# AustenLamacraft/audio-mps

Measured on AMD Instinct MI355X. Metric: audio samples/sec (fwd+bwd) at D=32, T=16000, higher is better.
Workload: dtype f32; 1 GPU; BASELINE configs[2]: PsiCMPS fwd+bwd scan, D=32, T=16000, batch 1024 per GPU (global 1024), input damped_sine, full optimiser step (device-resident chain rule + Adam); parallelism=dp1, kernel_variant=2, kernel_family=wave, input=damped_sine, optimizer_step=device (cmps_psi_apply_step), rank1_updates=f16x2

## Files before the change

audio_mps_amd/build.py:

```python
from __future__ import annotations

import os
import shutil
import subprocess
import sys

_HERE = os.path.dirname(os.path.abspath(__file__))
CSRC = os.path.join(_HERE, "csrc")
LIB_DIR = os.path.join(_HERE, "lib")
LIB_PATH = os.path.join(LIB_DIR, "libcmps.so")
OBJ_DIR = os.path.join(_HERE, "obj")
SOURCES = ["cmps_capi.hip", "cmps_prep.hip", "cmps_opt.hip", "cmps_block.hip", "cmps_wave.hip", "cmps_wave_bwd2.hip", "cmps_wave2.hip", "cmps_wave16.hip", "cmps_pair.hip", "cmps_wide.hip", "cmps_legacy.hip", "cmps_rho.hip", "cmps_rho_wave.hip", "cmps_rho_mfma.hip"]
EXTRA_FLAGS = {"cmps_pair.hip": ["-fno-slp-vectorize"]}
HEADERS = ["cmps_internal.h", "cmps_wave_util.h", "cmps_grad_gemm.h", os.path.join("..", "..", "include", "cmps.h")]


def _hipcc() -> str:
    for cand in (shutil.which("hipcc"), "/opt/rocm/bin/hipcc"):
        if cand and os.path.exists(cand):
            return cand
    raise RuntimeError("hipcc not found: libcmps.so cannot be built")


def needs_build() -> bool:
    if not os.path.exists(LIB_PATH):
        return True
    t = os.path.getmtime(LIB_PATH)
    deps = [os.path.join(CSRC, s) for s in SOURCES + HEADERS]
    return any(os.path.getmtime(d) > t for d in deps if os.path.exists(d))


def _flags():
    return ["--offload-arch=gfx950", "-O3", "-std=c++17", "-fPIC", "-Xarch_host", "-msse4.2", "-Wall", "-Wno-unused-function"]


def _stamp_text(flags) -> str:
    return " ".join(flags) + " | " + " ; ".join(f"{k}: {' '.join(v)}" for k, v in sorted(EXTRA_FLAGS.items()))


def build(force: bool = False, verbose: bool = False, extra_flags=(), jobs: int | None = None) -> str:
    import hashlib
    flags = _flags() + list(extra_flags)
    obj_dir, lib_path = OBJ_DIR, LIB_PATH
    if extra_flags:
        tag = hashlib.sha1(" ".join(extra_flags).encode()).hexdigest()[:10]
        obj_dir, lib_path = OBJ_DIR + "_diag_" + tag, os.path.join(LIB_DIR, f"libcmps_diag_{tag}.so")
    stamp = os.path.join(obj_dir, "flags.txt")
    same_flags = os.path.exists(stamp) and open(stamp).read() == _stamp_text(flags)
    if not force and not extra_flags and same_flags and not needs_build():
        return LIB_PATH
    os.makedirs(LIB_DIR, exist_ok=True)
    os.makedirs(obj_dir, exist_ok=True)
    hipcc = _hipcc()
    hdr_t = max(os.path.getmtime(os.path.join(CSRC, h)) for h in HEADERS if os.path.exists(os.path.join(CSRC, h)))
    todo, objs = [], []
    for s in SOURCES:
        src, obj = os.path.join(CSRC, s), os.path.join(obj_dir, s.replace(".hip", ".o"))
        objs.append(obj)
        if force or not same_flags or not os.path.exists(obj) or os.path.getmtime(obj) < max(os.path.getmtime(src), hdr_t):
            todo.append((src, obj))

    def compile_one(job):
        src, obj = job
        tmp = f"{obj}.{os.getpid()}.tmp"
        cmd = [hipcc] + flags + EXTRA_FLAGS.get(os.path.basename(src), []) + ["-c", src, "-o", tmp]
        if verbose:
            print(" ".join(cmd), file=sys.stderr)
        proc = subprocess.run(cmd, stdout=subprocess.PIPE, stderr=subprocess.STDOUT, text=True)
        if proc.returncode == 0:
            os.replace(tmp, obj)
        return src, proc

    from concurrent.futures import ThreadPoolExecutor
    with ThreadPoolExecutor(max_workers=jobs or min(6, os.cpu_count() or 2)) as pool:
        for src, proc in pool.map(compile_one, todo):
            if proc.returncode != 0:
                raise RuntimeError(f"hipcc failed on {src}:\n" + proc.stdout)
            if verbose and proc.stdout:
                print(proc.stdout, file=sys.stderr)
    with open(stamp, "w") as f:
        f.write(_stamp_text(flags))
    tmp_lib = f"{lib_path}.{os.getpid()}.tmp"
    proc = subprocess.run([hipcc, "--offload-arch=gfx950", "-shared", "-fPIC", "-o", tmp_lib] + objs,
                          stdout=subprocess.PIPE, stderr=subprocess.STDOUT, text=True)
    if proc.returncode != 0:
        raise RuntimeError("hipcc link failed:\n" + proc.stdout)
    os.replace(tmp_lib, lib_path)
    return lib_path


if __name__ == "__main__":
    print(build(force="--force" in sys.argv, verbose=True))
```

audio_mps_amd/csrc/cmps_wave_bwd2.hip:

```cpp
#include "cmps_wave_util.h"

namespace cmps {

namespace {

struct Pre2 {
    float yh, yho, yhp, un, pre;
    v2f rho;
    v2f sd;
    float inv, ten, rad;
};

constexpr int RING_SLOT = 256;
constexpr int RING_VAL = 8 * RING_SLOT;
constexpr int RING_HALF = 3 * RING_VAL;
constexpr int SPIN_MAX = 1 << 22;
constexpr int MT = 4;

__device__ __forceinline__ int flag_load2(unsigned addr) {
    int v;
    asm volatile("ds_read_b32 %0, %1\n\ts_waitcnt lgkmcnt(0)" : "=v"(v) : "v"(addr) : "memory");
    return __builtin_amdgcn_readfirstlane(v);
}
__device__ __forceinline__ void flag_store2(unsigned addr_l, int v) {
    asm volatile("ds_write_b32 %0, %1" : : "v"(addr_l), "v"(v) : "memory");
}
__device__ __forceinline__ void swap_fill(float& a, float& b, v2f& m0, v2f r0, v2f q0, v2f& m1, v2f r1, v2f q1, v2f s2) {
    asm("v_pk_fma_f32 %2, %4, %8, %5 op_sel_hi:[1,0,1]\n\t"
        "v_pk_fma_f32 %3, %6, %8, %7 op_sel_hi:[1,0,1]\n\t"
        "v_permlane32_swap_b32 %0, %1"
        : "+v"(a), "+v"(b), "=&v"(m0), "=&v"(m1) : "v"(r0), "v"(q0), "v"(r1), "v"(q1), "v"(s2));
}
template <int OFF>
__device__ __forceinline__ void ring_write(unsigned addr, float v) {
    asm volatile("ds_write_b32 %0, %1 offset:%2" : : "v"(addr), "v"(v), "n"(OFF) : "memory");
}
__device__ __forceinline__ float wave_max(float x) {
    asm("s_nop 1\n\tv_max_f32_dpp %0, %0, %0 quad_perm:[1,0,3,2] row_mask:0xf bank_mask:0xf\n\t"
        "s_nop 1\n\tv_max_f32_dpp %0, %0, %0 quad_perm:[2,3,0,1] row_mask:0xf bank_mask:0xf\n\t"
        "s_nop 1\n\tv_max_f32_dpp %0, %0, %0 row_half_mirror row_mask:0xf bank_mask:0xf\n\t"
        "s_nop 1\n\tv_max_f32_dpp %0, %0, %0 row_mirror row_mask:0xf bank_mask:0xf\n\t"
        "s_nop 1\n\tv_max_f32_dpp %0, %0, %0 row_bcast:15 row_mask:0xa bank_mask:0xf\n\t"
        "s_nop 1\n\tv_max_f32_dpp %0, %0, %0 row_bcast:31 row_mask:0xc bank_mask:0xf" : "+v"(x));
    return rdlane(x, 63);
}

}

__global__ __launch_bounds__(128 * WAVES, 1) void k_bwd_wave2w(Dev P, const float* __restrict__ audio) {
    __shared__ __attribute__((aligned(16))) float4 stY[WAVES][CHB * 32];
    __shared__ __attribute__((aligned(16))) float4 stR[WAVES][CHB * 16];
    __shared__ __attribute__((aligned(16))) float4 scl[WAVES][CH * 2];
    __shared__ __attribute__((aligned(16))) float2 bcB[WAVES][DPW];
    __shared__ __attribute__((aligned(16))) float ring[WAVES][2 * 3 * 8 * 64];
    __shared__ __attribute__((aligned(8))) float2 sct[WAVES][2][CH];
    __shared__ int flags[WAVES][2];
    __shared__ int flag_sink[WAVES][2][64];
    const int wv = __builtin_amdgcn_readfirstlane(threadIdx.x >> 6), lane = threadIdx.x & 63;
    const int w = wv & (WAVES - 1), role = wv / WAVES;
    const int i = lane & 31, h = lane >> 5;
    const bool hb = h != 0;
    if (threadIdx.x < 2 * WAVES) (&flags[0][0])[threadIdx.x] = 0;
    __syncthreads();
    const int b = blockIdx.x * WAVES + w;
    if (b >= P.B) return;
    const int N = P.N, T = P.T, NC = (N + CH - 1) / CH;
    const int u_top = (N - 1) & 7, a_oct = (N - 1 - u_top) >> 3, n_oct = (u_top ? 1 : 0) + a_oct + 1;
    const unsigned aProd = lds_addr(&flags[w][0]), aCons = lds_addr(&flags[w][1]);
    const unsigned aProdL = lane == 0 ? aProd : lds_addr(&flag_sink[w][0][lane]), aConsL = lane == 0 ? aCons : lds_addr(&flag_sink[w][1][lane]);
    const unsigned aRing0 = lds_addr(&ring[w][0]) + lane * 4;
    const int vr = P.phi0 ? P.phi_rank : 1;
    const int bc = b / vr, av = b - bc * vr;
    const float* xrow = audio + (size_t)bc * T;
    const float* sc = P.scal + scal_off(bc, NC, 0);
    const float A = dev_A(P);
    float* slab = P.slabs + (size_t)b * P.slab_floats;
    constexpr int DD = DPW * DPW;

    if (role == 0) {
        __builtin_amdgcn_s_setprio(3);
        stagger(w);
        v2f MRd[16], MQ[16], MM[16];
#pragma unroll
        for (int m = 0; m < 16; ++m) {
            const v2f rt = ld2(&P.RT[i * DPW + 16 * h + m]);
            MRd[m] = mk2(rt.x, -rt.y);
            MQ[m] = ld2(&P.Q[i * DPW + 16 * h + m]);
        }
        const unsigned aBw = lds_addr(&bcB[w][0]) + i * 8 + h * 4, aBr = lds_addr(&bcB[w][0]) + h * 128;
        const unsigned aYown = lds_addr(&stY[w][0]) + (2 * i + h) * 8;
        const unsigned aRho = lds_addr(&stR[w][0]) + i * 8;
        const unsigned aScl = lds_addr(&scl[w][0]);
        const float4* rho4 = reinterpret_cast<const float4*>(P.rho);
        const float4* sty4 = reinterpret_cast<const float4*>(P.hst + ((size_t)bc * N * vr + av) * 128);
        float facc = 0.f, accS = 0.f, accA = 0.f;
        float ra0 = 0.f, ra1 = 0.f, rdt = 0.f, rnv = 1.f, rev = 0.f;
        v4f so4[4], so2[2];
        auto octet_load = [&](int hh, int q) {
            stage_load512<4>(sty4, hh * CHB + 8 * q, N - 1, lane, so4, vr);
            stage_load<2>(rho4, hh * CHB + 8 * q, N, lane, so2);
        };
        const unsigned so_lane16 = (unsigned)lane * 16u;
        auto octet_load_below = [&](int hh, int q) {
            if (vr == 1) {
                const int row0 = __builtin_amdgcn_readfirstlane(hh * CHB + 8 * q);
                const float4* py = sty4 + (size_t)row0 * 32;
                const float4* pr = rho4 + (size_t)row0 * 16;
                asm volatile("global_load_dwordx4 %0, %6, %7\n\tglobal_load_dwordx4 %1, %6, %7 offset:1024\n\t"
                             "global_load_dwordx4 %2, %6, %7 offset:2048\n\tglobal_load_dwordx4 %3, %6, %7 offset:3072\n\t"
                             "global_load_dwordx4 %4, %6, %8\n\tglobal_load_dwordx4 %5, %6, %8 offset:1024"
                             : "=&v"(so4[0]), "=&v"(so4[1]), "=&v"(so4[2]), "=&v"(so4[3]), "=&v"(so2[0]), "=&v"(so2[1])
                             : "v"(so_lane16), "s"(py), "s"(pr) : "memory");
            } else {
                octet_load(hh, q);
            }
        };
        auto octet_commit = [&](int q) {
            stage_commit<4>(&stY[w][q * 256], lane, so4);
            stage_commit<2>(&stR[w][q * 128], lane, so2);
        };
        auto octet_commit_below = [&](int q) {
            asm volatile("s_waitcnt vmcnt(0)" : "+v"(so4[0]), "+v"(so4[1]), "+v"(so4[2]), "+v"(so4[3]), "+v"(so2[0]), "+v"(so2[1]) : : "memory");
            octet_commit(q);
        };
        auto scal_load = [&](int c) {
            const int idx = c * CH + lane;
            ra0 = idx < T ? xrow[idx] : 0.f;
            ra1 = idx + 1 < T ? xrow[idx + 1] : 0.f;
            rdt = P.dtk[idx];
            rnv = sc[(size_t)c * 128 + lane];
            rev = sc[(size_t)c * 128 + 64 + lane];
        };
        auto scal_commit = [&](int c) {
            const int idx = c * CH + lane;
            const float inc = ra1 - ra0;
            const float nv = rnv, ev = rev;
            const float invv = rsq_nr(fmaxf(nv, 1e-12f));
            const float invokv = nv > 1e-12f ? invv : 0.f;
            const float sv = inc / A;
            const float ex = ev * inc;
            const float z = ex / A;
            const float zbar = -1.0f / (1.0f + z);
            const float ebar = zbar * inc / A;
            const float tev = 2.0f * ebar;
            scl[w][2 * lane] = make_float4(sv, rdt, invv, tev * nv);
            scl[w][2 * lane + 1] = make_float4(tev, invokv, tev * ev, 0.f);
            sct[w][c & 1][lane] = make_float2(sv, tev * nv);
            if (idx < N) accA += zbar * ex;
        };
        auto make_pre = [&](v2f yh2, v2f rho, v4f c0, v4f c1, v2f sfill) -> Pre2 {
            const float yown = yh2.x, hown = yh2.y;
            Pre2 S;
            S.rho = rho;
            S.sd = __builtin_shufflevector(c0, c0, 0, 1);
            S.inv = c0.z;
            S.ten = c0.w;
            const float te = c1.x;
            const float invok = c1.y;
            S.rad = c1.z;
            S.pre = te * hown;
            S.yh = S.inv * yown;
            S.yhp = invok * yown;
            {
                float ya = S.yh, yb = S.yh;
                swap_fill(ya, yb, MM[10], MRd[10], MQ[10], MM[11], MRd[11], MQ[11], sfill);
                S.yho = hb ? -ya : yb;
            }
            const v2f un = cmul2(mk2(S.yh, S.yho), rho);
            S.un = un.x;
            return S;
        };

        const int hl = (N - 1) / CHB;
#pragma unroll 1
        for (int q = 0; q < 4; ++q) { octet_load(hl, q); octet_commit(q); }
        scal_load(hl >> 1);
        scal_commit(hl >> 1);
        v4f qc[8];
        v2f yh_j, rho_j;
        v4f c0_j, c1_j;
        Pre2 S;
        {
            const int jr = (N - 1) & (CHB - 1), jc = (N - 1) & (CH - 1);
            own_issue(aYown + jr * 512, aRho + jr * 256, aScl + jc * 32, yh_j, rho_j, c0_j, c1_j);
            lds_wait_own<0>(yh_j, rho_j, c0_j, c1_j);
            S = make_pre(yh_j, rho_j, c0_j, c1_j, __builtin_shufflevector(c0_j, c0_j, 0, 1));
        }
        {
            const v2f s2 = mk2(S.sd.x, S.sd.x);
#pragma unroll
            for (int m = 16 - MT; m < 16; ++m) MM[m] = __builtin_elementwise_fma(MRd[m], s2, MQ[m]);
        }
        float g = 0.f, go = 0.f;
        const float2 p0 = P.phi0 ? P.phi0[av * DPW + i] : P.psi0[i];
        const float u0 = hb ? p0.y : p0.x;
        float rad_next = 0.f;

        auto chain_step = [&](const Pre2& S, float uk, auto have_pre, bool exact, unsigned aslot, auto slot_off) -> Pre2 {
            constexpr int SO = decltype(slot_off)::value;
            facc += S.sd.y * (go * S.un);
            const v2f yhbp = cmul2_conj_b(mk2(g, go), S.rho);
            const float yhb = yhbp.x;
            float dot = rad_next;
            if (exact) {
                asm volatile("" ::: "memory");
                dot = sum64(S.yhp * yhb);
            }
            rad_next = S.rad;
            const float ybar = (yhb - dot * S.yhp) * S.inv + S.pre;
            bcast_issue(aBw, aBr, ybar, qc);
            {
                const v2f s2 = mk2(S.sd.x, S.sd.x);
#pragma unroll
                for (int m = 0; m < 16 - MT - 2; ++m) MM[m] = __builtin_elementwise_fma(MRd[m], s2, MQ[m]);
            }
            Pre2 Sn = S;
            if constexpr (!decltype(have_pre)::value) {
                const v2f s2 = mk2(S.sd.x, S.sd.x);
                MM[10] = __builtin_elementwise_fma(MRd[10], s2, MQ[10]);
                MM[11] = __builtin_elementwise_fma(MRd[11], s2, MQ[11]);
            }
            if constexpr (decltype(have_pre)::value) {
                lds_wait_own<9>(yh_j, rho_j, c0_j, c1_j);
                Sn = make_pre(yh_j, rho_j, c0_j, c1_j, S.sd);
                uk = Sn.un;
            }
            ring_write<SO>(aslot, ybar);
            ring_write<SO + RING_VAL>(aslot, S.yh);
            ring_write<SO + 2 * RING_VAL>(aslot, uk);
            lds_wait_lo<4 + 3>(qc);
            v2f am;
            mv1_lo(MM, qc, am);
            lds_wait_hi<3>(qc);
            mv1_hi(MM, qc, am);
            const v2f sn2 = __builtin_shufflevector(c0_j, c0_j, 0, 1);
            float sx = am.x, sy = am.y;
            swap_fill(sx, sy, MM[12], MRd[12], MQ[12], MM[13], MRd[13], MQ[13], sn2);
            const float md = sx + sy;
            accS += md * uk;
            g = ybar + md;
            float ga = g, gb = g;
            swap_fill(ga, gb, MM[14], MRd[14], MQ[14], MM[15], MRd[15], MQ[15], sn2);
            go = hb ? -ga : gb;
            return Sn;
        };
        int oct = 0;
        auto half_base = [&](int o) { return aRing0 + (unsigned)(o & 1) * RING_HALF; };
        int cons_seen = 0;
        auto peek_cons = [&]() {
            asm volatile("ds_read_b32 %0, %1" : "=v"(cons_seen) : "v"(aCons) : "memory");
        };
        auto wait_free = [&](int o) {
            int seen;
            asm volatile("s_nop 0\n\tv_readfirstlane_b32 %0, %1" : "=s"(seen) : "v"(cons_seen));
            if (o >= 2 && seen < o - 1) {
                int spin = 0;
                while (flag_load2(aCons) < o - 1 && ++spin < SPIN_MAX) __builtin_amdgcn_s_sleep(1);
            }
        };
        auto publish = [&]() {
            ++oct;
            flag_store2(aProdL, oct);
        };

        const bool proj_ok = P.phi0 == nullptr;
        if (hl >= 1) {
            const int jtop = N - 2, q_hi = jtop >= hl * CHB ? (jtop & (CHB - 1)) >> 3 : -1;
#pragma unroll 1
            for (int q = q_hi + 1; q < 4; ++q) { octet_load(hl - 1, q); octet_commit(q); }
        }
        if (u_top) {
            const unsigned ab = half_base(0);
            for (int t = 0; t < 8 - u_top; ++t) {
                asm volatile("ds_write_b32 %0, %1\n\tds_write_b32 %0, %1 offset:%2\n\tds_write_b32 %0, %1 offset:%3"
                             : : "v"(ab + t * RING_SLOT), "v"(0.f), "n"(RING_VAL), "n"(2 * RING_VAL) : "memory");
            }
        }
        for (int hh = hl; hh >= 0; --hh) {
            const int jlo = hh * CHB;
            const int jhi = (N - 2) < (jlo + CHB - 1) ? (N - 2) : (jlo + CHB - 1);
            const bool new_scal = (hh & 1) == 0 && hh > 0;
            if (new_scal) scal_load((hh >> 1) - 1);
            int j = jhi;
            if (j >= jlo && (j & 7) != 7) {
                const unsigned ab = half_base(0);
                const int q = (j & (CHB - 1)) >> 3;
                if (hh > 0) octet_load(hh - 1, q);
                int t = 8 - u_top;
                for (; j >= jlo && (j & 7) != 7; --j, ++t) {
                    const int jr = j & (CHB - 1), jc = j & (CH - 1);
                    own_issue(aYown + jr * 512, aRho + jr * 256, aScl + jc * 32, yh_j, rho_j, c0_j, c1_j);
                    S = chain_step(S, 0.f, std::true_type{}, proj_ok && j == jhi, ab + t * RING_SLOT, std::integral_constant<int, 0>{});
                }
                if (hh > 0) octet_commit(q);
                publish();
            }
#define BWD2_STEP8(PQ)                                                                                         \
            {                                                                                                 \
                if ((PQ) == 3) peek_cons();                                                                                \
                own_issue_off<(PQ) * 512, (PQ) * 256, (PQ) * 32>(aYo8, aRo8, aSo8, yh_j, rho_j, c0_j, c1_j);  \
                S = chain_step(S, 0.f, std::true_type{}, (PQ) == 7 && proj_ok && j == jhi, ab8, std::integral_constant<int, (7 - (PQ)) * RING_SLOT>{}); \
            }
            for (; j >= jlo; j -= 8) {
                const int q = (j & (CHB - 1)) >> 3;
                if (hh > 0) octet_load_below(hh - 1, q);
                wait_free(oct);
                const unsigned ab8 = half_base(oct);
                const unsigned aYo8 = aYown + ((j - 7) & (CHB - 1)) * 512, aRo8 = aRho + ((j - 7) & (CHB - 1)) * 256;
                const unsigned aSo8 = aScl + ((j - 7) & (CH - 1)) * 32;
                BWD2_STEP8(7) BWD2_STEP8(6) BWD2_STEP8(5) BWD2_STEP8(4) BWD2_STEP8(3) BWD2_STEP8(2) BWD2_STEP8(1) BWD2_STEP8(0)
                if (hh > 0) octet_commit_below(q);
                publish();
            }
#undef BWD2_STEP8
            if (new_scal) scal_commit((hh >> 1) - 1);
        }
        {
            wait_free(oct);
            const unsigned ab = half_base(oct);
            S = chain_step(S, u0, std::false_type{}, proj_ok, ab, std::integral_constant<int, 0>{});
            for (int t = 1; t < 8; ++t) {
                asm volatile("ds_write_b32 %0, %1\n\tds_write_b32 %0, %1 offset:%2\n\tds_write_b32 %0, %1 offset:%3"
                             : : "v"(ab + t * RING_SLOT), "v"(0.f), "n"(RING_VAL), "n"(2 * RING_VAL) : "memory");
            }
            publish();
        }
        const float sumS = sum64(accS);
        const float sumA = av == 0 ? sum64(accA) : 0.f;
        const float ftot = swapadd(facc, facc);
        slab[4 * DD + (hb ? 2 * DPW : DPW) + i] = g;
        if (!hb) slab[4 * DD + i] = ftot;
        if (lane == 0) {
            slab[4 * DD + 3 * DPW] = -(sumA / (A * A)) - sumS / A;
            slab[4 * DD + 3 * DPW + 1] = 0.f;
        }
        return;
    }

    __builtin_amdgcn_s_setprio(0);
    typedef _Float16 hf8 __attribute__((ext_vector_type(8)));
    typedef _Float16 hf2 __attribute__((ext_vector_type(2)));
    v16f Rre = {}, Rim = {}, Qre = {}, Qim = {};
    constexpr float SB16 = 8192.f;
    float sR = 1.f, sQ = 1.f;
    auto pow2_of = [](float bound) {
        int se = 12 - ((int)((__float_as_uint(bound) >> 23) & 0xFFu) - 126);
        se = se > 60 ? 60 : se < -60 ? -60 : se;
        return __uint_as_float((unsigned)(127 + se) << 23);
    };
    auto pow2_inv = [](float s2) { return __uint_as_float(0x7F000000u - __float_as_uint(s2)); };
    const unsigned aPart = lds_addr(&ring[w][0]) + (lane ^ 32) * 4;
    const unsigned aSct0 = lds_addr(&sct[w][0][0]);
    for (int o = 0; o < n_oct; ++o) {
        {
            int spin = 0;
            while (flag_load2(aProd) < o + 1 && ++spin < SPIN_MAX) __builtin_amdgcn_s_sleep(2);
        }
        const unsigned ab = aRing0 + (unsigned)(o & 1) * RING_HALF, ap = aPart + (unsigned)(o & 1) * RING_HALF;
        const int ktop = (u_top && o == 0) ? (N - 1) + (8 - u_top) : (o == n_oct - 1) ? 0 : (N - 1 - u_top) - 8 * (o - (u_top ? 1 : 0));
        int kl = ktop - (lane & 7);
        kl = kl < 0 ? 0 : (kl > N - 1 ? N - 1 : kl);
        const unsigned aSct = aSct0 + (unsigned)(((kl >> 6) & 1) * CH + (kl & (CH - 1))) * 8;
        float yb[8], yh[8], yhq[8], uu[8], uq[8];
        v2f stv;
#pragma unroll
        for (int t = 0; t < 8; t += 2) {
            asm volatile("ds_read2st64_b32 %0, %5 offset0:%7 offset1:%8\n\tds_read2st64_b32 %1, %5 offset0:%9 offset1:%10\n\t"
                         "ds_read2st64_b32 %2, %6 offset0:%9 offset1:%10\n\tds_read2st64_b32 %3, %5 offset0:%11 offset1:%12\n\t"
                         "ds_read2st64_b32 %4, %6 offset0:%11 offset1:%12"
                         : "=&v"(*reinterpret_cast<v2f*>(&yb[t])), "=&v"(*reinterpret_cast<v2f*>(&yh[t])), "=&v"(*reinterpret_cast<v2f*>(&yhq[t])),
                           "=&v"(*reinterpret_cast<v2f*>(&uu[t])), "=&v"(*reinterpret_cast<v2f*>(&uq[t]))
                         : "v"(ab), "v"(ap), "n"(t), "n"(t + 1), "n"(8 + t), "n"(8 + t + 1), "n"(16 + t), "n"(16 + t + 1) : "memory");
        }
        asm volatile("ds_read_b64 %0, %1" : "=&v"(stv) : "v"(aSct) : "memory");
        asm volatile("s_waitcnt lgkmcnt(0)" : "+v"(yb[0]), "+v"(yb[1]), "+v"(yb[2]), "+v"(yb[3]), "+v"(yb[4]), "+v"(yb[5]), "+v"(yb[6]), "+v"(yb[7]) :: "memory");
        asm volatile("s_waitcnt lgkmcnt(0)" : "+v"(yh[0]), "+v"(yh[1]), "+v"(yh[2]), "+v"(yh[3]), "+v"(yh[4]), "+v"(yh[5]), "+v"(yh[6]), "+v"(yh[7]) :: "memory");
        asm volatile("s_waitcnt lgkmcnt(0)" : "+v"(yhq[0]), "+v"(yhq[1]), "+v"(yhq[2]), "+v"(yhq[3]), "+v"(yhq[4]), "+v"(yhq[5]), "+v"(yhq[6]), "+v"(yhq[7]) :: "memory");
        asm volatile("s_waitcnt lgkmcnt(0)" : "+v"(uu[0]), "+v"(uu[1]), "+v"(uu[2]), "+v"(uu[3]), "+v"(uu[4]), "+v"(uu[5]), "+v"(uu[6]), "+v"(uu[7]) :: "memory");
        asm volatile("s_waitcnt lgkmcnt(0)" : "+v"(uq[0]), "+v"(uq[1]), "+v"(uq[2]), "+v"(uq[3]), "+v"(uq[4]), "+v"(uq[5]), "+v"(uq[6]), "+v"(uq[7]), "+v"(stv) :: "memory");
        flag_store2(aConsL, o + 1);
        float a1[8], a2[8], mQ = 0.f, mR = 0.f;
#pragma unroll
        for (int t = 0; t < 8; ++t) {
            const float sk = rdlane(stv.x, t), tn = rdlane(stv.y, t);
            a1[t] = tn * yh[t];
            a2[t] = sk * yb[t];
            mQ = fmaxf(mQ, fabsf(yb[t]));
            mR = fmaxf(mR, fmaxf(fabsf(a1[t]), fabsf(a2[t])));
        }
        mQ = wave_max(mQ);
        mR = wave_max(mR);
        {
            const float xq = mQ * sQ, xr = mR * sR;
            const bool chQ = mQ > 0.f && !(xq >= 32.f && xq < 32768.f), chR = mR > 0.f && !(xr >= 32.f && xr < 32768.f);
            if (chQ || chR) {
                const float nQ = chQ ? pow2_of(mQ) : sQ, nR = chR ? pow2_of(mR) : sR;
                const float fQ = nQ * pow2_inv(sQ), fR = nR * pow2_inv(sR);
#pragma unroll
                for (int r = 0; r < 16; ++r) { Rre[r] *= fR; Rim[r] *= fR; Qre[r] *= fQ; Qim[r] *= fQ; }
                sQ = nQ; sR = nR;
            }
        }
        unsigned fH[7][4], fL[7][4];
        auto split_pair = [&](int v, int reg, float ve, float vo, float sc2) {
            const v2f t = mk2(ve, vo) * mk2(sc2, sc2);
            const hf2 hh = {(_Float16)t.x, (_Float16)t.y};
            const unsigned H = __builtin_bit_cast(unsigned, hh);
            float re, ro;
            asm("v_fma_mix_f32 %0, %2, %4, -%5 op_sel:[0,0,0] op_sel_hi:[0,0,1]\n\t"
                "v_fma_mix_f32 %1, %3, %4, -%5 op_sel:[0,0,1] op_sel_hi:[0,0,1]"
                : "=&v"(re), "=&v"(ro) : "v"(ve), "v"(vo), "v"(sc2), "v"(H));
            const hf2 ll = {(_Float16)re, (_Float16)ro};
            fH[v][reg] = H;
            fL[v][reg] = __builtin_bit_cast(unsigned, ll);
        };
        const float sgB = hb ? -SB16 : SB16;
#pragma unroll
        for (int r = 0; r < 4; ++r) {
            split_pair(0, r, a1[2 * r], a1[2 * r + 1], sR);
            split_pair(1, r, yb[2 * r], yb[2 * r + 1], sQ);
            split_pair(2, r, a2[2 * r], a2[2 * r + 1], sR);
            split_pair(3, r, yh[2 * r], yh[2 * r + 1], SB16);
            split_pair(4, r, yhq[2 * r], yhq[2 * r + 1], sgB);
            split_pair(5, r, uu[2 * r], uu[2 * r + 1], SB16);
            split_pair(6, r, uq[2 * r], uq[2 * r + 1], sgB);
        }
        auto frag = [&](const unsigned (&f)[4]) { return __builtin_bit_cast(hf8, v4u{f[0], f[1], f[2], f[3]}); };
        auto mf3 = [&](v16f& acc, int ia, int ib) {
            acc = __builtin_amdgcn_mfma_f32_32x32x16_f16(frag(fH[ia]), frag(fH[ib]), acc, 0, 0, 0);
            acc = __builtin_amdgcn_mfma_f32_32x32x16_f16(frag(fH[ia]), frag(fL[ib]), acc, 0, 0, 0);
            acc = __builtin_amdgcn_mfma_f32_32x32x16_f16(frag(fL[ia]), frag(fH[ib]), acc, 0, 0, 0);
        };
        mf3(Rre, 0, 3);
        mf3(Rim, 0, 4);
        mf3(Qre, 1, 5);
        mf3(Qim, 1, 6);
        mf3(Rre, 2, 5);
        mf3(Rim, 2, 6);
    }
    const float uR = pow2_inv(sR) * (1.0f / SB16), uQ = pow2_inv(sQ) * (1.0f / SB16);
#pragma unroll
    for (int r = 0; r < 16; ++r) {
        const int row = (r & 3) + 8 * (r >> 2) + 4 * h;
        const int oo = row * DPW + i;
        slab[oo] = Rre[r] * uR;
        slab[DD + oo] = -Rim[r] * uR;
        slab[2 * DD + oo] = Qre[r] * uQ;
        slab[3 * DD + oo] = -Qim[r] * uQ;
    }
}

hipError_t launch_bwd_wave2w(const Dev& P, const float* audio, hipStream_t s) {
    const unsigned nb = (unsigned)((P.B + WAVES - 1) / WAVES);
    hipLaunchKernelGGL(k_bwd_wave2w, dim3(nb), dim3(128 * WAVES), 0, s, P, audio);
    return hipGetLastError();
}

}
```

Before: 1.706 billion samples/s.

## Move u and force-accumulation work from backward chain wave to consumer wave

Strips the u = rho·yh products, the swap_fill for yho, and the facc/accS accumulations out of the latency-critical serial chain_step in the producer wave. The consumer wave now rebuilds them from the ring (yh, md) plus rho loaded directly through buffer loads, and reads scalar coefficients from a reorganised sct layout. It also merges the two wave-max reductions into one interleaved DPP sequence and disables SLP vectorisation for the file. This shortens the serial recurrence at the cost of more work and global loads in the consumer, plus an extra LDS handoff for sumA.

Result: no change. 1.719 billion samples/s, median of 6 (+0.8%).

```diff
diff --git a/audio_mps_amd/build.py b/audio_mps_amd/build.py
--- a/audio_mps_amd/build.py
+++ b/audio_mps_amd/build.py
@@ -11,7 +11,7 @@
 LIB_PATH = os.path.join(LIB_DIR, "libcmps.so")
 OBJ_DIR = os.path.join(_HERE, "obj")
 SOURCES = ["cmps_capi.hip", "cmps_prep.hip", "cmps_opt.hip", "cmps_block.hip", "cmps_wave.hip", "cmps_wave_bwd2.hip", "cmps_wave2.hip", "cmps_wave16.hip", "cmps_pair.hip", "cmps_wide.hip", "cmps_legacy.hip", "cmps_rho.hip", "cmps_rho_wave.hip", "cmps_rho_mfma.hip"]
-EXTRA_FLAGS = {"cmps_pair.hip": ["-fno-slp-vectorize"]}
+EXTRA_FLAGS = {"cmps_pair.hip": ["-fno-slp-vectorize"], "cmps_wave_bwd2.hip": ["-fno-slp-vectorize"]}
 HEADERS = ["cmps_internal.h", "cmps_wave_util.h", "cmps_grad_gemm.h", os.path.join("..", "..", "include", "cmps.h")]
 
 
diff --git a/audio_mps_amd/csrc/cmps_wave_bwd2.hip b/audio_mps_amd/csrc/cmps_wave_bwd2.hip
--- a/audio_mps_amd/csrc/cmps_wave_bwd2.hip
+++ b/audio_mps_amd/csrc/cmps_wave_bwd2.hip
@@ -5,7 +5,7 @@
 namespace {
 
 struct Pre2 {
-    float yh, yho, yhp, un, pre;
+    float yh, yhp, pre;
     v2f rho;
     v2f sd;
     float inv, ten, rad;
@@ -15,6 +15,7 @@
 constexpr int RING_VAL = 8 * RING_SLOT;
 constexpr int RING_HALF = 3 * RING_VAL;
 constexpr int SPIN_MAX = 1 << 22;
+constexpr int SCT = 2 * CH + 8;
 constexpr int MT = 4;
 
 __device__ __forceinline__ int flag_load2(unsigned addr) {
@@ -35,14 +36,17 @@
 __device__ __forceinline__ void ring_write(unsigned addr, float v) {
     asm volatile("ds_write_b32 %0, %1 offset:%2" : : "v"(addr), "v"(v), "n"(OFF) : "memory");
 }
-__device__ __forceinline__ float wave_max(float x) {
-    asm("s_nop 1\n\tv_max_f32_dpp %0, %0, %0 quad_perm:[1,0,3,2] row_mask:0xf bank_mask:0xf\n\t"
-        "s_nop 1\n\tv_max_f32_dpp %0, %0, %0 quad_perm:[2,3,0,1] row_mask:0xf bank_mask:0xf\n\t"
-        "s_nop 1\n\tv_max_f32_dpp %0, %0, %0 row_half_mirror row_mask:0xf bank_mask:0xf\n\t"
-        "s_nop 1\n\tv_max_f32_dpp %0, %0, %0 row_mirror row_mask:0xf bank_mask:0xf\n\t"
-        "s_nop 1\n\tv_max_f32_dpp %0, %0, %0 row_bcast:15 row_mask:0xa bank_mask:0xf\n\t"
-        "s_nop 1\n\tv_max_f32_dpp %0, %0, %0 row_bcast:31 row_mask:0xc bank_mask:0xf" : "+v"(x));
-    return rdlane(x, 63);
+__device__ __forceinline__ void wave_max2(float& x, float& y) {
+    asm("s_nop 1\n\t"
+        "v_max_f32_dpp %0, %0, %0 quad_perm:[1,0,3,2] row_mask:0xf bank_mask:0xf\n\tv_max_f32_dpp %1, %1, %1 quad_perm:[1,0,3,2] row_mask:0xf bank_mask:0xf\n\ts_nop 0\n\t"
+        "v_max_f32_dpp %0, %0, %0 quad_perm:[2,3,0,1] row_mask:0xf bank_mask:0xf\n\tv_max_f32_dpp %1, %1, %1 quad_perm:[2,3,0,1] row_mask:0xf bank_mask:0xf\n\ts_nop 0\n\t"
+        "v_max_f32_dpp %0, %0, %0 row_half_mirror row_mask:0xf bank_mask:0xf\n\tv_max_f32_dpp %1, %1, %1 row_half_mirror row_mask:0xf bank_mask:0xf\n\ts_nop 0\n\t"
+        "v_max_f32_dpp %0, %0, %0 row_mirror row_mask:0xf bank_mask:0xf\n\tv_max_f32_dpp %1, %1, %1 row_mirror row_mask:0xf bank_mask:0xf\n\ts_nop 0\n\t"
+        "v_max_f32_dpp %0, %0, %0 row_bcast:15 row_mask:0xa bank_mask:0xf\n\tv_max_f32_dpp %1, %1, %1 row_bcast:15 row_mask:0xa bank_mask:0xf\n\ts_nop 0\n\t"
+        "v_max_f32_dpp %0, %0, %0 row_bcast:31 row_mask:0xc bank_mask:0xf\n\tv_max_f32_dpp %1, %1, %1 row_bcast:31 row_mask:0xc bank_mask:0xf"
+        : "+v"(x), "+v"(y));
+    x = rdlane(x, 63);
+    y = rdlane(y, 63);
 }
 
 }
@@ -53,7 +57,8 @@
     __shared__ __attribute__((aligned(16))) float4 scl[WAVES][CH * 2];
     __shared__ __attribute__((aligned(16))) float2 bcB[WAVES][DPW];
     __shared__ __attribute__((aligned(16))) float ring[WAVES][2 * 3 * 8 * 64];
-    __shared__ __attribute__((aligned(8))) float2 sct[WAVES][2][CH];
+    __shared__ __attribute__((aligned(16))) float sct[WAVES][2][SCT];
+    __shared__ float xfer[WAVES];
     __shared__ int flags[WAVES][2];
     __shared__ int flag_sink[WAVES][2][64];
     const int wv = __builtin_amdgcn_readfirstlane(threadIdx.x >> 6), lane = threadIdx.x & 63;
@@ -61,11 +66,12 @@
     const int i = lane & 31, h = lane >> 5;
     const bool hb = h != 0;
     if (threadIdx.x < 2 * WAVES) (&flags[0][0])[threadIdx.x] = 0;
+    for (int e = threadIdx.x; e < WAVES * 2 * SCT; e += 128 * WAVES) (&sct[0][0][0])[e] = 0.f;
     __syncthreads();
     const int b = blockIdx.x * WAVES + w;
     if (b >= P.B) return;
     const int N = P.N, T = P.T, NC = (N + CH - 1) / CH;
-    const int u_top = (N - 1) & 7, a_oct = (N - 1 - u_top) >> 3, n_oct = (u_top ? 1 : 0) + a_oct + 1;
+    const int u_top = (N - 1) & 7, a_oct = (N - 1 - u_top) >> 3, n_oct = 1 + a_oct + 1;
     const unsigned aProd = lds_addr(&flags[w][0]), aCons = lds_addr(&flags[w][1]);
     const unsigned aProdL = lane == 0 ? aProd : lds_addr(&flag_sink[w][0][lane]), aConsL = lane == 0 ? aCons : lds_addr(&flag_sink[w][1][lane]);
     const unsigned aRing0 = lds_addr(&ring[w][0]) + lane * 4;
@@ -93,7 +99,7 @@
         const unsigned aScl = lds_addr(&scl[w][0]);
         const float4* rho4 = reinterpret_cast<const float4*>(P.rho);
         const float4* sty4 = reinterpret_cast<const float4*>(P.hst + ((size_t)bc * N * vr + av) * 128);
-        float facc = 0.f, accS = 0.f, accA = 0.f;
+        float accA = 0.f;
         float ra0 = 0.f, ra1 = 0.f, rdt = 0.f, rnv = 1.f, rev = 0.f;
         v4f so4[4], so2[2];
         auto octet_load = [&](int hh, int q) {
@@ -145,10 +151,14 @@
             const float tev = 2.0f * ebar;
             scl[w][2 * lane] = make_float4(sv, rdt, invv, tev * nv);
             scl[w][2 * lane + 1] = make_float4(tev, invokv, tev * ev, 0.f);
-            sct[w][c & 1][lane] = make_float2(sv, tev * nv);
+            const int pos = (120 - idx) & (2 * CH - 1);
+            const float svk = idx < N ? sv : 0.f, tnk = idx < N ? tev * nv : 0.f;
+            sct[w][0][pos] = svk;
+            sct[w][1][pos] = tnk;
+            if (pos < 8) { sct[w][0][pos + 2 * CH] = svk; sct[w][1][pos + 2 * CH] = tnk; }
             if (idx < N) accA += zbar * ex;
         };
-        auto make_pre = [&](v2f yh2, v2f rho, v4f c0, v4f c1, v2f sfill) -> Pre2 {
+        auto make_pre = [&](v2f yh2, v2f rho, v4f c0, v4f c1) -> Pre2 {
             const float yown = yh2.x, hown = yh2.y;
             Pre2 S;
             S.rho = rho;
@@ -161,13 +171,6 @@
             S.pre = te * hown;
             S.yh = S.inv * yown;
             S.yhp = invok * yown;
-            {
-                float ya = S.yh, yb = S.yh;
-                swap_fill(ya, yb, MM[10], MRd[10], MQ[10], MM[11], MRd[11], MQ[11], sfill);
-                S.yho = hb ? -ya : yb;
-            }
-            const v2f un = cmul2(mk2(S.yh, S.yho), rho);
-            S.un = un.x;
             return S;
         };
 
@@ -184,7 +187,7 @@
             const int jr = (N - 1) & (CHB - 1), jc = (N - 1) & (CH - 1);
             own_issue(aYown + jr * 512, aRho + jr * 256, aScl + jc * 32, yh_j, rho_j, c0_j, c1_j);
             lds_wait_own<0>(yh_j, rho_j, c0_j, c1_j);
-            S = make_pre(yh_j, rho_j, c0_j, c1_j, __builtin_shufflevector(c0_j, c0_j, 0, 1));
+            S = make_pre(yh_j, rho_j, c0_j, c1_j);
         }
         {
             const v2f s2 = mk2(S.sd.x, S.sd.x);
@@ -192,13 +195,10 @@
             for (int m = 16 - MT; m < 16; ++m) MM[m] = __builtin_elementwise_fma(MRd[m], s2, MQ[m]);
         }
         float g = 0.f, go = 0.f;
-        const float2 p0 = P.phi0 ? P.phi0[av * DPW + i] : P.psi0[i];
-        const float u0 = hb ? p0.y : p0.x;
         float rad_next = 0.f;
 
-        auto chain_step = [&](const Pre2& S, float uk, auto have_pre, bool exact, unsigned aslot, auto slot_off) -> Pre2 {
+        auto chain_step = [&](const Pre2& S, auto have_pre, bool exact, unsigned aslot, auto slot_off) -> Pre2 {
             constexpr int SO = decltype(slot_off)::value;
-            facc += S.sd.y * (go * S.un);
             const v2f yhbp = cmul2_conj_b(mk2(g, go), S.rho);
             const float yhb = yhbp.x;
             float dot = rad_next;
@@ -212,36 +212,30 @@
             {
                 const v2f s2 = mk2(S.sd.x, S.sd.x);
 #pragma unroll
-                for (int m = 0; m < 16 - MT - 2; ++m) MM[m] = __builtin_elementwise_fma(MRd[m], s2, MQ[m]);
+                for (int m = 0; m < 16 - MT; ++m) MM[m] = __builtin_elementwise_fma(MRd[m], s2, MQ[m]);
             }
             Pre2 Sn = S;
-            if constexpr (!decltype(have_pre)::value) {
-                const v2f s2 = mk2(S.sd.x, S.sd.x);
-                MM[10] = __builtin_elementwise_fma(MRd[10], s2, MQ[10]);
-                MM[11] = __builtin_elementwise_fma(MRd[11], s2, MQ[11]);
-            }
+            float yh_below = 0.f;
             if constexpr (decltype(have_pre)::value) {
                 lds_wait_own<9>(yh_j, rho_j, c0_j, c1_j);
-                Sn = make_pre(yh_j, rho_j, c0_j, c1_j, S.sd);
-                uk = Sn.un;
+                Sn = make_pre(yh_j, rho_j, c0_j, c1_j);
+                yh_below = Sn.yh;
             }
             ring_write<SO>(aslot, ybar);
-            ring_write<SO + RING_VAL>(aslot, S.yh);
-            ring_write<SO + 2 * RING_VAL>(aslot, uk);
-            lds_wait_lo<4 + 3>(qc);
+            ring_write<SO + RING_VAL>(aslot, yh_below);
+            lds_wait<2>(qc);
             v2f am;
             mv1_lo(MM, qc, am);
-            lds_wait_hi<3>(qc);
             mv1_hi(MM, qc, am);
             const v2f sn2 = __builtin_shufflevector(c0_j, c0_j, 0, 1);
             float sx = am.x, sy = am.y;
             swap_fill(sx, sy, MM[12], MRd[12], MQ[12], MM[13], MRd[13], MQ[13], sn2);
             const float md = sx + sy;
-            accS += md * uk;
             g = ybar + md;
             float ga = g, gb = g;
             swap_fill(ga, gb, MM[14], MRd[14], MQ[14], MM[15], MRd[15], MQ[15], sn2);
             go = hb ? -ga : gb;
+            ring_write<SO + 2 * RING_VAL>(aslot, md);
             return Sn;
         };
         int oct = 0;
@@ -269,12 +263,14 @@
 #pragma unroll 1
             for (int q = q_hi + 1; q < 4; ++q) { octet_load(hl - 1, q); octet_commit(q); }
         }
-        if (u_top) {
+        {
             const unsigned ab = half_base(0);
             for (int t = 0; t < 8 - u_top; ++t) {
-                asm volatile("ds_write_b32 %0, %1\n\tds_write_b32 %0, %1 offset:%2\n\tds_write_b32 %0, %1 offset:%3"
-                             : : "v"(ab + t * RING_SLOT), "v"(0.f), "n"(RING_VAL), "n"(2 * RING_VAL) : "memory");
-            }
+                const float yv = t == 7 - u_top ? S.yh : 0.f;
+                asm volatile("ds_write_b32 %0, %1\n\tds_write_b32 %0, %2 offset:%3\n\tds_write_b32 %0, %1 offset:%4"
+                             : : "v"(ab + t * RING_SLOT), "v"(0.f), "v"(yv), "n"(RING_VAL), "n"(2 * RING_VAL) : "memory");
+            }
+            if (!u_top) publish();
         }
         for (int hh = hl; hh >= 0; --hh) {
             const int jlo = hh * CHB;
@@ -290,7 +286,7 @@
                 for (; j >= jlo && (j & 7) != 7; --j, ++t) {
                     const int jr = j & (CHB - 1), jc = j & (CH - 1);
                     own_issue(aYown + jr * 512, aRho + jr * 256, aScl + jc * 32, yh_j, rho_j, c0_j, c1_j);
-                    S = chain_step(S, 0.f, std::true_type{}, proj_ok && j == jhi, ab + t * RING_SLOT, std::integral_constant<int, 0>{});
+                    S = chain_step(S, std::true_type{}, proj_ok && j == jhi, ab + t * RING_SLOT, std::integral_constant<int, 0>{});
                 }
                 if (hh > 0) octet_commit(q);
                 publish();
@@ -299,7 +295,7 @@
             {                                                                                                 \
                 if ((PQ) == 3) peek_cons();                                                                                \
                 own_issue_off<(PQ) * 512, (PQ) * 256, (PQ) * 32>(aYo8, aRo8, aSo8, yh_j, rho_j, c0_j, c1_j);  \
-                S = chain_step(S, 0.f, std::true_type{}, (PQ) == 7 && proj_ok && j == jhi, ab8, std::integral_constant<int, (7 - (PQ)) * RING_SLOT>{}); \
+                S = chain_step(S, std::true_type{}, (PQ) == 7 && proj_ok && j == jhi, ab8, std::integral_constant<int, (7 - (PQ)) * RING_SLOT>{}); \
             }
             for (; j >= jlo; j -= 8) {
                 const int q = (j & (CHB - 1)) >> 3;
@@ -318,22 +314,17 @@
         {
             wait_free(oct);
             const unsigned ab = half_base(oct);
-            S = chain_step(S, u0, std::false_type{}, proj_ok, ab, std::integral_constant<int, 0>{});
+            S = chain_step(S, std::false_type{}, proj_ok, ab, std::integral_constant<int, 0>{});
             for (int t = 1; t < 8; ++t) {
                 asm volatile("ds_write_b32 %0, %1\n\tds_write_b32 %0, %1 offset:%2\n\tds_write_b32 %0, %1 offset:%3"
                              : : "v"(ab + t * RING_SLOT), "v"(0.f), "n"(RING_VAL), "n"(2 * RING_VAL) : "memory");
             }
+            const float sumA = av == 0 ? sum64(accA) : 0.f;
+            asm volatile("ds_write_b32 %0, %1" : : "v"(lds_addr(&xfer[w])), "v"(-(sumA / (A * A))) : "memory");
             publish();
         }
-        const float sumS = sum64(accS);
-        const float sumA = av == 0 ? sum64(accA) : 0.f;
-        const float ftot = swapadd(facc, facc);
         slab[4 * DD + (hb ? 2 * DPW : DPW) + i] = g;
-        if (!hb) slab[4 * DD + i] = ftot;
-        if (lane == 0) {
-            slab[4 * DD + 3 * DPW] = -(sumA / (A * A)) - sumS / A;
-            slab[4 * DD + 3 * DPW + 1] = 0.f;
-        }
+        if (lane == 0) slab[4 * DD + 3 * DPW + 1] = 0.f;
         return;
     }
 
@@ -351,45 +342,89 @@
     auto pow2_inv = [](float s2) { return __uint_as_float(0x7F000000u - __float_as_uint(s2)); };
     const unsigned aPart = lds_addr(&ring[w][0]) + (lane ^ 32) * 4;
     const unsigned aSct0 = lds_addr(&sct[w][0][0]);
+    const float sgn = hb ? -1.f : 1.f;
+    float facc = 0.f, accS = 0.f;
+    float cU = 0.f, cGq = 0.f;
+    const __amdgpu_buffer_rsrc_t rhoR = __builtin_amdgcn_make_buffer_rsrc((void*)P.rho, (short)0, (N + 1) * DPW * 8, 0x00020000);
+    const float2 p0 = P.phi0 ? P.phi0[av * DPW + i] : P.psi0[i];
+    const float pU = hb ? p0.y : p0.x, pUq = hb ? p0.x : p0.y;
+    typedef __attribute__((address_space(4))) const float cfloat;
+    cfloat* dtkc = (cfloat*)P.dtk;
     for (int o = 0; o < n_oct; ++o) {
         {
             int spin = 0;
             while (flag_load2(aProd) < o + 1 && ++spin < SPIN_MAX) __builtin_amdgcn_s_sleep(2);
         }
         const unsigned ab = aRing0 + (unsigned)(o & 1) * RING_HALF, ap = aPart + (unsigned)(o & 1) * RING_HALF;
-        const int ktop = (u_top && o == 0) ? (N - 1) + (8 - u_top) : (o == n_oct - 1) ? 0 : (N - 1 - u_top) - 8 * (o - (u_top ? 1 : 0));
-        int kl = ktop - (lane & 7);
-        kl = kl < 0 ? 0 : (kl > N - 1 ? N - 1 : kl);
-        const unsigned aSct = aSct0 + (unsigned)(((kl >> 6) & 1) * CH + (kl & (CH - 1))) * 8;
-        float yb[8], yh[8], yhq[8], uu[8], uq[8];
-        v2f stv;
+        const int ktop = o == 0 ? (N - 1) + (8 - u_top) : (o == n_oct - 1) ? 0 : (N - 1 - u_top) - 8 * (o - 1);
+        const unsigned aSct = aSct0 + (unsigned)((120 - ktop) & (2 * CH - 1)) * 4;
+        v2f rr[8];
+        float dts[8];
+        {
+            unsigned vro = (unsigned)(ktop - 8) * (DPW * 8) + (unsigned)i * 8;
+            asm volatile("" : "+v"(vro));
+            const int kb = ktop >= 7 ? ktop - 7 : 0;
+#pragma unroll
+            for (int t = 0; t < 8; ++t) {
+                rr[t] = __builtin_bit_cast(v2f, __builtin_amdgcn_raw_buffer_load_b64(rhoR, vro + (7 - t) * (DPW * 8), 0, 0));
+                dts[t] = dtkc[kb + 7 - t];
+            }
+            if (ktop == 0) dts[0] = dtkc[0];
+        }
+        float yb[8], ybq[8], Y[8], Yq[8], md[8], mdq[8];
+        v4f st4[2];
+        v2f tn2[4];
 #pragma unroll
         for (int t = 0; t < 8; t += 2) {
-            asm volatile("ds_read2st64_b32 %0, %5 offset0:%7 offset1:%8\n\tds_read2st64_b32 %1, %5 offset0:%9 offset1:%10\n\t"
-                         "ds_read2st64_b32 %2, %6 offset0:%9 offset1:%10\n\tds_read2st64_b32 %3, %5 offset0:%11 offset1:%12\n\t"
-                         "ds_read2st64_b32 %4, %6 offset0:%11 offset1:%12"
-                         : "=&v"(*reinterpret_cast<v2f*>(&yb[t])), "=&v"(*reinterpret_cast<v2f*>(&yh[t])), "=&v"(*reinterpret_cast<v2f*>(&yhq[t])),
-                           "=&v"(*reinterpret_cast<v2f*>(&uu[t])), "=&v"(*reinterpret_cast<v2f*>(&uq[t]))
+            asm volatile("ds_read2st64_b32 %0, %6 offset0:%8 offset1:%9\n\tds_read2st64_b32 %1, %7 offset0:%8 offset1:%9\n\t"
+                         "ds_read2st64_b32 %2, %6 offset0:%10 offset1:%11\n\tds_read2st64_b32 %3, %7 offset0:%10 offset1:%11\n\t"
+                         "ds_read2st64_b32 %4, %6 offset0:%12 offset1:%13\n\tds_read2st64_b32 %5, %7 offset0:%12 offset1:%13"
+                         : "=&v"(*reinterpret_cast<v2f*>(&yb[t])), "=&v"(*reinterpret_cast<v2f*>(&ybq[t])), "=&v"(*reinterpret_cast<v2f*>(&Y[t])),
+                           "=&v"(*reinterpret_cast<v2f*>(&Yq[t])), "=&v"(*reinterpret_cast<v2f*>(&md[t])), "=&v"(*reinterpret_cast<v2f*>(&mdq[t]))
                          : "v"(ab), "v"(ap), "n"(t), "n"(t + 1), "n"(8 + t), "n"(8 + t + 1), "n"(16 + t), "n"(16 + t + 1) : "memory");
         }
-        asm volatile("ds_read_b64 %0, %1" : "=&v"(stv) : "v"(aSct) : "memory");
+        asm volatile("ds_read_b128 %0, %6\n\tds_read_b128 %1, %6 offset:16\n\t"
+                     "ds_read2_b32 %2, %6 offset0:%7 offset1:%8\n\tds_read2_b32 %3, %6 offset0:%9 offset1:%10\n\t"
+                     "ds_read2_b32 %4, %6 offset0:%11 offset1:%12\n\tds_read2_b32 %5, %6 offset0:%13 offset1:%14"
+                     : "=&v"(st4[0]), "=&v"(st4[1]), "=&v"(tn2[0]), "=&v"(tn2[1]), "=&v"(tn2[2]), "=&v"(tn2[3])
+                     : "v"(aSct), "n"(SCT + 1), "n"(SCT + 2), "n"(SCT + 3), "n"(SCT + 4), "n"(SCT + 5), "n"(SCT + 6), "n"(SCT + 7), "n"(SCT + 8)
+                     : "memory");
         asm volatile("s_waitcnt lgkmcnt(0)" : "+v"(yb[0]), "+v"(yb[1]), "+v"(yb[2]), "+v"(yb[3]), "+v"(yb[4]), "+v"(yb[5]), "+v"(yb[6]), "+v"(yb[7]) :: "memory");
-        asm volatile("s_waitcnt lgkmcnt(0)" : "+v"(yh[0]), "+v"(yh[1]), "+v"(yh[2]), "+v"(yh[3]), "+v"(yh[4]), "+v"(yh[5]), "+v"(yh[6]), "+v"(yh[7]) :: "memory");
-        asm volatile("s_waitcnt lgkmcnt(0)" : "+v"(yhq[0]), "+v"(yhq[1]), "+v"(yhq[2]), "+v"(yhq[3]), "+v"(yhq[4]), "+v"(yhq[5]), "+v"(yhq[6]), "+v"(yhq[7]) :: "memory");
-        asm volatile("s_waitcnt lgkmcnt(0)" : "+v"(uu[0]), "+v"(uu[1]), "+v"(uu[2]), "+v"(uu[3]), "+v"(uu[4]), "+v"(uu[5]), "+v"(uu[6]), "+v"(uu[7]) :: "memory");
-        asm volatile("s_waitcnt lgkmcnt(0)" : "+v"(uq[0]), "+v"(uq[1]), "+v"(uq[2]), "+v"(uq[3]), "+v"(uq[4]), "+v"(uq[5]), "+v"(uq[6]), "+v"(uq[7]), "+v"(stv) :: "memory");
+        asm volatile("s_waitcnt lgkmcnt(0)" : "+v"(ybq[0]), "+v"(ybq[1]), "+v"(ybq[2]), "+v"(ybq[3]), "+v"(ybq[4]), "+v"(ybq[5]), "+v"(ybq[6]), "+v"(ybq[7]) :: "memory");
+        asm volatile("s_waitcnt lgkmcnt(0)" : "+v"(Y[0]), "+v"(Y[1]), "+v"(Y[2]), "+v"(Y[3]), "+v"(Y[4]), "+v"(Y[5]), "+v"(Y[6]), "+v"(Y[7]) :: "memory");
+        asm volatile("s_waitcnt lgkmcnt(0)" : "+v"(Yq[0]), "+v"(Yq[1]), "+v"(Yq[2]), "+v"(Yq[3]), "+v"(Yq[4]), "+v"(Yq[5]), "+v"(Yq[6]), "+v"(Yq[7]) :: "memory");
+        asm volatile("s_waitcnt lgkmcnt(0)" : "+v"(md[0]), "+v"(md[1]), "+v"(md[2]), "+v"(md[3]), "+v"(md[4]), "+v"(md[5]), "+v"(md[6]), "+v"(md[7]) :: "memory");
+        asm volatile("s_waitcnt lgkmcnt(0)" : "+v"(mdq[0]), "+v"(mdq[1]), "+v"(mdq[2]), "+v"(mdq[3]), "+v"(mdq[4]), "+v"(mdq[5]), "+v"(mdq[6]), "+v"(mdq[7]),
+                     "+v"(st4[0]), "+v"(st4[1]), "+v"(tn2[0]), "+v"(tn2[1]), "+v"(tn2[2]), "+v"(tn2[3]) :: "memory");
         flag_store2(aConsL, o + 1);
+        float uu[8], uq[8], uc[8];
+#pragma unroll
+        for (int t = 0; t < 8; ++t) {
+            const float rs = sgn * rr[t].y;
+            uc[t] = Y[t] * rr[t].x - Yq[t] * rs;
+            uq[t] = Yq[t] * rr[t].x + Y[t] * rs;
+            uu[t] = uc[t];
+        }
+        if (o == n_oct - 1) { uu[0] = pU; uq[0] = pUq; }
+#pragma unroll
+        for (int t = 0; t < 8; ++t) {
+            const float gq = ybq[t] + mdq[t];
+            facc += dts[t] * (cGq * cU);
+            accS += md[t] * uu[t];
+            cGq = gq;
+            cU = uc[t];
+        }
+
         float a1[8], a2[8], mQ = 0.f, mR = 0.f;
 #pragma unroll
         for (int t = 0; t < 8; ++t) {
-            const float sk = rdlane(stv.x, t), tn = rdlane(stv.y, t);
-            a1[t] = tn * yh[t];
+            const float sk = st4[t >> 2][t & 3], tn = (t & 1) ? tn2[t >> 1].y : tn2[t >> 1].x;
+            a1[t] = tn * Y[t];
             a2[t] = sk * yb[t];
             mQ = fmaxf(mQ, fabsf(yb[t]));
             mR = fmaxf(mR, fmaxf(fabsf(a1[t]), fabsf(a2[t])));
         }
-        mQ = wave_max(mQ);
-        mR = wave_max(mR);
+        wave_max2(mQ, mR);
         {
             const float xq = mQ * sQ, xr = mR * sR;
             const bool chQ = mQ > 0.f && !(xq >= 32.f && xq < 32768.f), chR = mR > 0.f && !(xr >= 32.f && xr < 32768.f);
@@ -420,8 +455,8 @@
             split_pair(0, r, a1[2 * r], a1[2 * r + 1], sR);
             split_pair(1, r, yb[2 * r], yb[2 * r + 1], sQ);
             split_pair(2, r, a2[2 * r], a2[2 * r + 1], sR);
-            split_pair(3, r, yh[2 * r], yh[2 * r + 1], SB16);
-            split_pair(4, r, yhq[2 * r], yhq[2 * r + 1], sgB);
+            split_pair(3, r, Y[2 * r], Y[2 * r + 1], SB16);
+            split_pair(4, r, Yq[2 * r], Yq[2 * r + 1], sgB);
             split_pair(5, r, uu[2 * r], uu[2 * r + 1], SB16);
             split_pair(6, r, uq[2 * r], uq[2 * r + 1], sgB);
         }
@@ -437,6 +472,15 @@
         mf3(Qim, 1, 6);
         mf3(Rre, 2, 5);
         mf3(Rim, 2, 6);
+    }
+    {
+        const float sumS = sum64(accS);
+        const float fl = sgn * facc;
+        const float ftot = swapadd(fl, fl);
+        if (!hb) slab[4 * DD + i] = ftot;
+        float xa;
+        asm volatile("ds_read_b32 %0, %1\n\ts_waitcnt lgkmcnt(0)" : "=v"(xa) : "v"(lds_addr(&xfer[w])) : "memory");
+        if (lane == 0) slab[4 * DD + 3 * DPW] = xa - sumS / A;
     }
     const float uR = pow2_inv(sR) * (1.0f / SB16), uQ = pow2_inv(sQ) * (1.0f / SB16);
 #pragma unroll
```
